# qzwlecr/p1

Hardware: AMD Instinct MI355X
Metric: SHA-256 nonce-hashes/sec (GH/s) (higher is better)
Workload: dtype u32

## Files before the change

include/p1hip.h:

```cpp
#ifndef P1HIP_H
#define P1HIP_H

#include <stddef.h>
#include <stdint.h>

#ifdef __cplusplus
extern "C" {
#endif

#define P1HIP_OK 0
#define P1HIP_ERR_NO_DEVICE (-1)
#define P1HIP_ERR_HIP (-2)
#define P1HIP_ERR_RCCL (-3)
#define P1HIP_ERR_ARGS (-4)

#define P1HIP_MAX_MSG_LEN ((size_t)1 << 28)

int p1hip_init(int want_devices, int *got_devices);

int p1hip_init_devices(const int *ordinals, int n);

int p1hip_scan(const uint8_t *msg, size_t msg_len, uint64_t lower, uint64_t upper,
               uint64_t *out_hash, uint64_t *out_nonce);

// ... 23 lines not shown
  uint64_t tiles;
  uint64_t nonces;
  double wall_ms;
} p1hip_batch_stats_t;
int p1hip_get_batch_stats(p1hip_batch_stats_t *out);

int p1hip_scan_batch_wide(const p1hip_request_t *reqs, size_t n, p1hip_result_t *out);

int p1hip_wide_layout(const p1hip_request_t *reqs, size_t n, int ndev,
                      int32_t *route, int32_t *device, uint32_t *segs, uint32_t *tiles);

int p1hip_wide_ranges(const p1hip_request_t *reqs, size_t n, int ndev, size_t cap, size_t *count,
                      uint32_t *req, uint32_t *tile0, uint32_t *ntiles, int32_t *launch,
                      uint32_t *dev_tiles);

typedef struct {
  uint64_t calls;
  uint64_t requests;
  uint64_t empty;
  uint64_t small;
  uint64_t wide;
  uint64_t individual;
  uint64_t scan_launches;
  uint64_t scan_segments;
  uint64_t generic_launches;
  uint64_t generic_segments;
  uint64_t tiles;
  uint64_t nonces;
  double wall_ms;
} p1hip_wide_stats_t;
int p1hip_get_wide_stats(p1hip_wide_stats_t *out);

typedef struct {
  uint64_t scans;
  uint64_t fast_launches;
  uint64_t fast_nonces;
  uint64_t fast_alg_ops;
  uint64_t generic_launches;
  uint64_t generic_nonces;
  double scan_wall_ms;
  uint64_t scan_launches;
  uint64_t scan_nonces;
  uint64_t scan_alg_ops;
  double scan_kernel_ms;
  uint64_t small_scans;
  uint64_t table_replans;
} p1hip_stats_t;

typedef struct {
  int32_t ordinal;
  int32_t active;
  uint64_t shard_first;
  uint64_t shard_last;
  uint64_t scans;
  uint64_t scan_launches;
  uint64_t scan_nonces;
  uint64_t scan_alg_ops;
  double scan_kernel_ms;
  double phase1_ms;
  double gather_ms;
} p1hip_device_stats_t;

int p1hip_get_device_stats(int index, p1hip_device_stats_t *out);

int p1hip_set_profiling(int on);
int p1hip_get_stats(p1hip_stats_t *out);
// ... 34 lines not shown
```

p1_amd/__init__.py:

```python
from ._lib import (
    P1HipError,
    lib_path,
    load,
    init,
    init_devices,
    scan,
    scan_batch,
    batch_layout,
    get_batch_stats,
    scan_batch_wide,
    wide_layout,
    get_wide_stats,
    hash,
    reduce_pairs,
    plan_shards,
    set_profiling,
    get_stats,
    get_device_stats,
    reset_stats,
    device_count,
    device_info,
    comm_info,
    abi_version,
    ABI_VERSION,
    test_knobs,
    shutdown,
    version,
    codeobj_bytes,
    codeobj_sha256,
    batch_codeobj_sha256,
)
from .sharding import shard_range, combine_keys
```

p1_amd/_lib.py:

```python
import ctypes
import os

_HERE = os.path.dirname(os.path.abspath(__file__))
_LIB = None

U64 = ctypes.c_uint64


class P1HipError(RuntimeError):
    def __init__(self, rc, msg):
        super().__init__(f"p1hip rc={rc}: {msg}")
        self.rc = rc


class Stats(ctypes.Structure):
    _fields_ = [
        ("scans", U64),
        ("fast_launches", U64),
        ("fast_nonces", U64),
        ("fast_alg_ops", U64),
        ("generic_launches", U64),
        ("generic_nonces", U64),
        ("scan_wall_ms", ctypes.c_double),
        ("scan_launches", U64),
# ... 38 lines not shown
class BatchStats(ctypes.Structure):
    _fields_ = [
        ("calls", U64),
        ("requests", U64),
        ("coalesced", U64),
        ("individual", U64),
        ("empty", U64),
        ("launches", U64),
        ("tiles", U64),
        ("nonces", U64),
        ("wall_ms", ctypes.c_double),
    ]

    def as_dict(self):
        return {k: getattr(self, k) for k, _ in self._fields_}


class WideStats(ctypes.Structure):
    _fields_ = [
        ("calls", U64),
        ("requests", U64),
        ("empty", U64),
        ("small", U64),
        ("wide", U64),
        ("individual", U64),
        ("scan_launches", U64),
        ("scan_segments", U64),
        ("generic_launches", U64),
        ("generic_segments", U64),
        ("tiles", U64),
        ("nonces", U64),
        ("wall_ms", ctypes.c_double),
    ]

    def as_dict(self):
        return {k: getattr(self, k) for k, _ in self._fields_}


class DeviceInfo(ctypes.Structure):
    _fields_ = [
        ("ordinal", ctypes.c_int32),
        ("cu_count", ctypes.c_int32),
        ("clock_khz", ctypes.c_int32),
        ("reserved", ctypes.c_int32),
        ("hbm_bytes", U64),
        ("pci_bus_id", ctypes.c_char * 32),
        ("arch", ctypes.c_char * 32),
        ("uuid", ctypes.c_ubyte * 16),
    ]

    def as_dict(self):
        return {"ordinal": self.ordinal, "cu_count": self.cu_count, "clock_khz": self.clock_khz,
                "hbm_bytes": self.hbm_bytes, "pci_bus_id": self.pci_bus_id.decode(errors="replace"),
                "arch": self.arch.decode(errors="replace"), "uuid": bytes(self.uuid).hex()}


def lib_path():
    return os.environ.get("P1HIP_LIB") or os.path.join(_HERE, "libp1hip.so")


SIGNATURES = [
    ("p1hip_init", ctypes.c_int, [ctypes.c_int, ctypes.POINTER(ctypes.c_int)]),
    ("p1hip_init_devices", ctypes.c_int, [ctypes.POINTER(ctypes.c_int), ctypes.c_int]),
    ("p1hip_scan", ctypes.c_int,
     [ctypes.c_char_p, ctypes.c_size_t, U64, U64, ctypes.POINTER(U64), ctypes.POINTER(U64)]),
    ("p1hip_scan_batch", ctypes.c_int, [ctypes.POINTER(Request), ctypes.c_size_t, ctypes.POINTER(Result)]),
    ("p1hip_batch_layout", ctypes.c_int,
     [ctypes.POINTER(Request), ctypes.c_size_t, ctypes.c_int, ctypes.POINTER(ctypes.c_uint32),
      ctypes.POINTER(ctypes.c_int32), ctypes.POINTER(ctypes.c_int32)]),
    ("p1hip_get_batch_stats", ctypes.c_int, [ctypes.POINTER(BatchStats)]),
    ("p1hip_scan_batch_wide", ctypes.c_int, [ctypes.POINTER(Request), ctypes.c_size_t, ctypes.POINTER(Result)]),
    ("p1hip_wide_layout", ctypes.c_int,
     [ctypes.POINTER(Request), ctypes.c_size_t, ctypes.c_int, ctypes.POINTER(ctypes.c_int32),
      ctypes.POINTER(ctypes.c_int32), ctypes.POINTER(ctypes.c_uint32), ctypes.POINTER(ctypes.c_uint32)]),
    ("p1hip_wide_ranges", ctypes.c_int,
     [ctypes.POINTER(Request), ctypes.c_size_t, ctypes.c_int, ctypes.c_size_t, ctypes.POINTER(ctypes.c_size_t),
      ctypes.POINTER(ctypes.c_uint32), ctypes.POINTER(ctypes.c_uint32), ctypes.POINTER(ctypes.c_uint32),
      ctypes.POINTER(ctypes.c_int32), ctypes.POINTER(ctypes.c_uint32)]),
    ("p1hip_get_wide_stats", ctypes.c_int, [ctypes.POINTER(WideStats)]),
    ("p1hip_hash", ctypes.c_int, [ctypes.c_char_p, ctypes.c_size_t, U64, ctypes.POINTER(U64)]),
    ("p1hip_plan_shards", ctypes.c_int,
     [ctypes.c_char_p, ctypes.c_size_t, U64, U64, ctypes.c_int, ctypes.POINTER(U64), ctypes.POINTER(U64)]),
    ("p1hip_reduce_pairs", ctypes.c_int,
     [ctypes.POINTER(U64), ctypes.POINTER(U64), ctypes.c_size_t, ctypes.POINTER(U64), ctypes.POINTER(U64)]),
    ("p1hip_set_profiling", ctypes.c_int, [ctypes.c_int]),
    ("p1hip_get_stats", ctypes.c_int, [ctypes.POINTER(Stats)]),
    ("p1hip_reset_stats", None, []),
    ("p1hip_get_device_stats", ctypes.c_int, [ctypes.c_int, ctypes.POINTER(DeviceStats)]),
    ("p1hip_device_count", ctypes.c_int, []),
    ("p1hip_device_info", ctypes.c_int, [ctypes.c_int, ctypes.POINTER(DeviceInfo)]),
    ("p1hip_comm_info", ctypes.c_int, [ctypes.c_int, ctypes.POINTER(ctypes.c_int), ctypes.POINTER(ctypes.c_int)]),
    ("p1hip_abi_version", ctypes.c_int, []),
    ("p1hip_test_knobs", ctypes.c_char_p, []),
    ("p1hip_last_error", ctypes.c_char_p, []),
    ("p1hip_version", ctypes.c_char_p, []),
    ("p1hip_shutdown", None, []),
]


def load(path=None):
    global _LIB
    if _LIB is not None and path is None:
        return _LIB
    p = path or lib_path()
    if not os.path.exists(p):
        raise P1HipError(-100, f"{p} not built (run `make` or __graft_entry__.build())")
    lib = ctypes.CDLL(p)
    for name, res, args in SIGNATURES:
        fn = getattr(lib, name)
        fn.restype = res
        fn.argtypes = args
    if lib.p1hip_abi_version() != ABI_VERSION:
# ... 82 lines not shown
    _check(load().p1hip_wide_layout(arr, n, int(ndev), route, device, segs, tiles))
    lay = [{"route": WIDE_ROUTES[route[i]], "device": device[i], "segs": segs[i], "tiles": tiles[i], "ranges": []}
           for i in range(n)]
    cap = sum(x["segs"] + 1 for x in lay)
    count = ctypes.c_size_t(0)
    req, tile0, ntiles = ((ctypes.c_uint32 * max(cap, 1))() for _ in range(3))
    launch = (ctypes.c_int32 * max(cap, 1))()
    dev_tiles = (ctypes.c_uint32 * int(ndev))()
    _check(load().p1hip_wide_ranges(arr, n, int(ndev), cap, ctypes.byref(count), req, tile0, ntiles, launch,
                                    dev_tiles))
    assert count.value <= cap
    for j in range(count.value):
        lay[req[j]]["ranges"].append((tile0[j], ntiles[j], launch[j]))
    return lay, list(dev_tiles)


def get_wide_stats():
    s = WideStats()
    _check(load().p1hip_get_wide_stats(ctypes.byref(s)))
    return s.as_dict()


def batch_codeobj_sha256(lib=None):
    import hashlib

    lib = lib or load()
    start = ctypes.addressof(ctypes.c_char.in_dll(lib, "p1hip_batch_co"))
    end = ctypes.addressof(ctypes.c_char.in_dll(lib, "p1hip_batch_co_end"))
    if end <= start:
        raise P1HipError(-100, "embedded batch code object is empty")
    return hashlib.sha256(ctypes.string_at(start, end - start)).hexdigest()


def hash(msg, nonce):
    m = _bytes(msg)
    h = U64()
    _check(load().p1hip_hash(m, len(m), int(nonce), ctypes.byref(h)))
    return h.value


def plan_shards(msg, lower, upper, n):
    m = _bytes(msg)
    first, last = (U64 * n)(), (U64 * n)()
    _check(load().p1hip_plan_shards(m, len(m), int(lower), int(upper), int(n), first, last))
    return [(a, b) if a <= b else None for a, b in zip(first, last)]


def reduce_pairs(hashes, nonces):
    n = len(hashes)
    assert n == len(nonces)
    ha = (U64 * max(n, 1))(*hashes)
    na = (U64 * max(n, 1))(*nonces)
    h, o = U64(), U64()
    _check(load().p1hip_reduce_pairs(ha, na, n, ctypes.byref(h), ctypes.byref(o)))
    return h.value, o.value


def set_profiling(on):
    _check(load().p1hip_set_profiling(1 if on else 0))


def get_stats():
    s = Stats()
    _check(load().p1hip_get_stats(ctypes.byref(s)))
    return s.as_dict()

# ... 61 lines not shown
```

p1_amd/csrc/p1hip.hip:

```cpp
#include <hip/hip_runtime.h>
#include <rccl/rccl.h>

#include <stdlib.h>
#include <string.h>

#include <algorithm>
#include <atomic>
#include <chrono>
#include <exception>
#include <mutex>
#include <string>
#include <thread>
#include <utility>
#include <vector>

#include "../../include/p1hip.h"
#include "batch_plan.hpp"
#include "planner.hpp"
#include "scan_abi.hpp"
#include "scan_pack.hpp"
#include "wide_plan.hpp"

extern "C" const unsigned char p1hip_kernels_co[];
extern "C" const unsigned char p1hip_batch_co[];

using namespace p1;

namespace {

thread_local std::string g_err;

int fail(int rc, const std::string& what) {
  g_err = what;
  return rc;
}

template <typename Fn>
int guarded(Fn&& fn) {
  try {
    return fn();
  } catch (const std::exception& ex) {
    return fail(P1HIP_ERR_HIP, std::string("host: ") + ex.what());
  } catch (...) {
    return fail(P1HIP_ERR_HIP, "host: unknown exception");
  }
}

#define HIPCHK(expr)                                                                        \
  do {                                                                                      \
    hipError_t e_ = (expr);                                                                 \
    if (e_ != hipSuccess)                                                                   \
      return fail(P1HIP_ERR_HIP, std::string(#expr) + ": " + hipGetErrorString(e_));       \
  } while (0)

#define NCCLCHK(expr)                                                                       \
  do {                                                                                      \
    ncclResult_t r_ = (expr);                                                               \
    if (r_ != ncclSuccess)                                                                  \
      return fail(P1HIP_ERR_RCCL, std::string(#expr) + ": " + ncclGetErrorString(r_));      \
  } while (0)

constexpr size_t kMaxKwTabs = 8;
constexpr uint64_t kMaxKwTabBytes = 8ull << 30;
constexpr uint64_t kMaxScanSpan = 1ull << 40;

enum KnobKind { kValue, kZeroDef, kFlag };
enum KnobWhen { kPerScan, kPerBatch, kAtInit };
enum KnobId {
  kSmallMaxNoncesKnob, kMaxLaunchBlocksKnob, kMaxScanSpanKnob, kKwtabMaxBytesKnob, kNoRcclKnob, kForceRcclKnob,
  kMinFastThreadsKnob, kTestFailDeviceKnob, kNoTableKnob, kNoSplitKnob, kScanGridKnob, kBatchMaxNoncesKnob,
  kBatchMaxTilesKnob, kWideMaxNoncesKnob, kWideMaxSegsKnob, kWideMinFastThreadsKnob, kKnobCount
};
struct Knob {
  const char* name;
  uint64_t def, max;
  KnobKind kind;
  KnobWhen when;
  const char* what;
};
const Knob kKnobs[] = {
    {"P1HIP_SMALL_MAX_NONCES", kSmallMaxNonces, kSmallMaxNonces, kValue, kPerScan,
     "shares of at most this many nonces take the one-launch small path; 0 turns it off, so small parity ranges "
     "run the fast kernel variants"},
    {"P1HIP_MAX_LAUNCH_BLOCKS", kMaxLaunchBlocks, kMaxLaunchBlocks, kZeroDef, kPerScan,
     "workgroups per k_scan launch, so GPU tests run the multi-launch path on small ranges; a larger piece gets "
     "a launch of its own (at most kMaxFastThreads / kBlock = 2^18 workgroups, far below HIP's grid limit)"},
    {"P1HIP_MAX_SCAN_SPAN", kMaxScanSpan, ~0ull, kZeroDef, kPerScan, "nonces per piece of a device's share"},
    {"P1HIP_KWTAB_MAX_BYTES", kMaxKwTabBytes, ~0ull, kValue, kPerScan,
     "MODE 5 table cap; a larger table re-plans the share without MODE 5"},
    {"P1HIP_NO_RCCL", 0, 1, kFlag, kAtInit,
     "combine the per-device results through the host, so the multi-device path (threads, sharding, combine) "
     "runs with the same GPU listed twice on a 1-GPU box"},
    {"P1HIP_FORCE_RCCL", 0, 1, kFlag, kAtInit, "a communicator even for one device"},
    {"P1HIP_MIN_FAST_THREADS", kMinFastThreads, ~0ull, kValue, kAtInit,
     "planner occupancy floor; 1 keeps k = 3 on small ranges so every k = 3 variant runs on the GPU"},
    {"P1HIP_TEST_FAIL_DEVICE", ~0ull, ~0ull, kValue, kAtInit,
     "device index whose scan phase reports a failure (the multi-device error path); default -1: none"},
    {"P1HIP_NO_TABLE", 0, 1, kFlag, kAtInit,
     "no MODE 5: layouts whose tail block 1 holds only lo digits run the digit-update variants (A/B, and a "
     "second kernel path to cross-check MODE 5)"},
    {"P1HIP_NO_SPLIT", 0, 1, kFlag, kAtInit,
     "straddling lo digits use mode 2 instead of the split modes (A/B builds with -DP1_NV2_PLAIN)"},
    {"P1HIP_SCAN_GRID", 0, kMaxLaunchBlocks, kZeroDef, kPerScan,
     "k_scan's grid instead of the device's workgroup slots (the default, 0); at or above a launch's tile count "
     "every workgroup runs one tile and the queue hands out none (the round-5 dispatch, same code object)"},
    {"P1HIP_BATCH_MAX_NONCES", kBatchMaxNonces, kBatchMaxNonces, kValue, kPerBatch,
     "requests of at most this many nonces are coalesced by p1hip_scan_batch; 0 runs every request "
     "individually; independent of P1HIP_SMALL_MAX_NONCES"},
    {"P1HIP_BATCH_MAX_TILES", kBatchMaxTiles, kBatchMaxTiles, kZeroDef, kPerBatch,
     "tiles per launch pair, so GPU tests run several launch pairs on small batches (batch_layout raises it to "
     "the largest single request's tile count)"},
    {"P1HIP_WIDE_MAX_NONCES", kWideMaxNonces, kWideMaxNonces, kValue, kPerBatch,
     "requests above the coalescing limit and of at most this many nonces share k_scan launches in "
     "p1hip_scan_batch_wide; larger ones run individually (0: all of them)"},
    {"P1HIP_WIDE_MAX_SEGS", kMaxSegs, kMaxSegs, kZeroDef, kPerBatch,
     "segments per k_scan launch of p1hip_scan_batch_wide, so GPU tests run many launches back to back on small "
     "calls and requests whose pieces land in different launches"},
    {"P1HIP_WIDE_MIN_FAST_THREADS", 0, ~0ull, kZeroDef, kPerBatch,
     "occupancy floor the wide requests are planned with instead of wide_min_fast_threads' rule (the default, "
     "0); 1 keeps k = 3"},
};
static_assert(sizeof kKnobs / sizeof kKnobs[0] == kKnobCount, "one row per KnobId, in its order");

bool test_knobs_on() {
  const char* m = getenv("P1HIP_TEST_KNOBS");
  return m && m[0] == '1' && m[1] == 0;
}

const char* test_knob(const char* name) {
  if (!test_knobs_on()) return nullptr;
  const char* v = getenv(name);
  return v && *v ? v : nullptr;
}

uint64_t knob(KnobId id) {
  const Knob& K = kKnobs[id];
  const char* v = test_knob(K.name);
  if (!v) return K.def;
  if (K.kind == kFlag) return v[0] == '1';
  const uint64_t n = strtoull(v, nullptr, 10);
  if (n == 0 && K.kind == kZeroDef) return K.def;
  return n < K.max ? n : K.max;
}

template <typename T, bool kPinned>
struct Buf {
  T* p = nullptr;
  size_t cap = 0;

  Buf() = default;
  Buf(const Buf&) = delete;
  Buf(Buf&& o) noexcept : p(std::exchange(o.p, nullptr)), cap(std::exchange(o.cap, 0)) {}
  Buf& operator=(Buf&& o) noexcept {
    if (this != &o) {
      (void)release();
      p = std::exchange(o.p, nullptr);
      cap = std::exchange(o.cap, 0);
    }
    return *this;
  }
  ~Buf() { (void)release(); }

  hipError_t release() {
    hipError_t e = hipSuccess;
    if (p) e = kPinned ? hipHostFree(p) : hipFree(p);
    p = nullptr;
    cap = 0;
    return e;
  }
  hipError_t reserve(size_t need, size_t floor, size_t extra = 0) {
    if (need <= cap) return hipSuccess;
    hipError_t e = release();
    if (e != hipSuccess) return e;
    size_t n = floor;
    while (n < need) n <<= 1;
    const size_t bytes = (n + extra) * sizeof(T);
    e = kPinned ? hipHostMalloc(&p, bytes, hipHostMallocDefault) : hipMalloc(&p, bytes);
    if (e != hipSuccess) p = nullptr;
    else cap = n;
    return e;
  }
};
template <typename T> using DevBuf = Buf<T, false>;
template <typename T> using PinnedBuf = Buf<T, true>;

struct Dev {
  int ordinal = -1;
  hipStream_t stream = nullptr;
  DevBuf<Key> d_part;
  DevBuf<Key> d_res;
  DevBuf<Key> d_gather;
  PinnedBuf<Key> h_res;
  DevBuf<Segment> d_seg;
  PinnedBuf<Segment> h_seg;
  ncclComm_t comm = nullptr;
  hipModule_t mod = nullptr;
  hipFunction_t f_scan = nullptr, f_reduce = nullptr, f_pairs = nullptr, f_small = nullptr, f_kwtable = nullptr;
  DevBuf<Key> d_small_part;
  DevBuf<uint32_t> d_ticket;
  DevBuf<uint32_t> d_scan_ticket;
  uint32_t scan_grid = 0;
  bool small_used = false;
  hipModule_t bmod = nullptr;
  hipFunction_t f_bscan = nullptr, f_breduce = nullptr, f_wreduce = nullptr;
  DevBuf<BatchSeg> d_bseg;
  PinnedBuf<BatchSeg> h_bseg;
  DevBuf<uint32_t> d_btile0;
  PinnedBuf<uint32_t> h_btile0;
  DevBuf<Key> d_bout;
  PinnedBuf<Key> h_bout;
  DevBuf<Key> d_bpart;
  DevBuf<WideRange> d_wrange;
  PinnedBuf<WideRange> h_wrange;
  std::vector<hipEvent_t> evs;
  struct KwTab {
    uint32_t w[16];
    int k;
    uint32_t* dptr;
    uint64_t used_in;
  };
  std::vector<KwTab> kwtabs;
  uint64_t range_id = 0;
  ScanCounters ctr;
  uint64_t replans = 0;
  p1hip_device_stats_t acc{};
};

struct Runtime {
  std::mutex mu;
  std::vector<Dev> devs;
  bool profiling = false;
  bool use_rccl = true;
  bool rccl_one = false;
  uint64_t min_fast_threads = kMinFastThreads;
  bool split = true;
  bool tabulate = true;
  int fail_device = -1;
  p1hip_stats_t stats{};
  p1hip_batch_stats_t bstats{};
  p1hip_wide_stats_t wstats{};
};

Runtime& rt() {
  static Runtime* r = new Runtime();
  return *r;
}

int device_count(int* count) {
  *count = 0;
  if (hipGetDeviceCount(count) != hipSuccess || *count <= 0)
    return fail(P1HIP_ERR_NO_DEVICE, "no HIP device visible");
  return P1HIP_OK;
}

template <typename... Args>
hipError_t launch(hipFunction_t f, uint32_t blocks, uint32_t threads, hipStream_t st, Args... args) {
  void* params[] = {(void*)&args...};
  return hipModuleLaunchKernel(f, blocks, 1, 1, threads, 1, 1, 0, st, params, nullptr);
}

int ev_record(Dev& d, size_t& nev) {
  if (d.evs.size() <= nev) {
    hipEvent_t e;
    HIPCHK(hipEventCreate(&e));
    d.evs.push_back(e);
  }
  HIPCHK(hipEventRecord(d.evs[nev], d.stream));
  ++nev;
  return P1HIP_OK;
}

int ev_sum(Dev& d, size_t nev) {
  if (!nev) return P1HIP_OK;
// ... 11 lines not shown
  return k;
}

void add_counters(p1hip_stats_t& s, const ScanCounters& c) {
  s.fast_launches += c.fast_launches;
  s.fast_nonces += c.fast_nonces;
  s.fast_alg_ops += c.fast_ops;
  s.generic_launches += c.gen_launches;
  s.generic_nonces += c.gen_nonces;
  s.scan_launches += c.scan_launches;
  s.scan_nonces += c.scan_nonces;
  s.scan_alg_ops += c.scan_ops;
  s.scan_kernel_ms += c.scan_ms;
}

void add_counters(p1hip_device_stats_t& a, const ScanCounters& c) {
  a.scans++;
  a.scan_launches += c.scan_launches;
  a.scan_nonces += c.scan_nonces;
  a.scan_alg_ops += c.scan_ops;
  a.scan_kernel_ms += c.scan_ms;
}

int dev_release(Dev& d) {
  if (d.ordinal < 0) return 0;
  (void)hipSetDevice(d.ordinal);
  if (d.stream) (void)hipStreamSynchronize(d.stream);
  for (hipEvent_t e : d.evs) (void)hipEventDestroy(e);
  for (Dev::KwTab& t : d.kwtabs) (void)hipFree(t.dptr);
  if (d.comm) ncclCommDestroy(d.comm);
  if (d.stream) (void)hipStreamDestroy(d.stream);
  if (d.mod) (void)hipModuleUnload(d.mod);
  if (d.bmod) (void)hipModuleUnload(d.bmod);
  d = Dev();
  return 0;
}

void shutdown_locked(Runtime& R) {
  for (Dev& d : R.devs) dev_release(d);
  R.devs.clear();
}

int init_devs(Runtime& R, const std::vector<int>& ords) {
  int count = 0;
  if (int rc = device_count(&count)) return rc;
  const int nd = (int)ords.size();
  std::vector<int> cus(ords.size());
  for (int i = 0; i < nd; ++i) {
    const int o = ords[i];
    if (o < 0 || o >= count) return fail(P1HIP_ERR_NO_DEVICE, "device ordinal out of range: " + std::to_string(o));
    hipDeviceProp_t prop;
    HIPCHK(hipGetDeviceProperties(&prop, o));
    if (std::string(prop.gcnArchName).rfind("gfx950", 0) != 0)
      return fail(P1HIP_ERR_NO_DEVICE, std::string("device is not gfx950: ") + prop.gcnArchName);
    cus[i] = prop.multiProcessorCount;
  }
  R.devs.resize(ords.size());
  for (int i = 0; i < nd; ++i) {
    Dev& d = R.devs[i];
    d.ordinal = ords[i];
    HIPCHK(hipSetDevice(d.ordinal));
    HIPCHK(hipStreamCreateWithFlags(&d.stream, hipStreamNonBlocking));
    HIPCHK(hipModuleLoadData(&d.mod, p1hip_kernels_co));
    HIPCHK(hipModuleGetFunction(&d.f_scan, d.mod, "k_scan"));
    HIPCHK(hipModuleGetFunction(&d.f_reduce, d.mod, "k_reduce"));
    HIPCHK(hipModuleGetFunction(&d.f_pairs, d.mod, "k_pairs"));
    HIPCHK(hipModuleGetFunction(&d.f_small, d.mod, "k_scan_small"));
    HIPCHK(hipModuleGetFunction(&d.f_kwtable, d.mod, "k_kwtable"));
    HIPCHK(hipModuleLoadData(&d.bmod, p1hip_batch_co));
    HIPCHK(hipModuleGetFunction(&d.f_bscan, d.bmod, "k_batch_scan"));
    HIPCHK(hipModuleGetFunction(&d.f_breduce, d.bmod, "k_batch_reduce"));
    HIPCHK(hipModuleGetFunction(&d.f_wreduce, d.bmod, "k_wide_reduce"));
    HIPCHK(d.d_small_part.reserve(kSmallMaxBlocks, kSmallMaxBlocks));
    HIPCHK(d.d_ticket.reserve(1, 1));
    HIPCHK(d.d_scan_ticket.reserve(2, 2));
    HIPCHK(hipMemsetAsync(d.d_ticket.p, 0, sizeof(uint32_t), d.stream));
    HIPCHK(hipMemsetAsync(d.d_scan_ticket.p, 0, 2 * sizeof(uint32_t), d.stream));
    int per_cu = 0;
    HIPCHK(hipModuleOccupancyMaxActiveBlocksPerMultiprocessor(&per_cu, d.f_scan, kBlock, 0));
    if (per_cu < 1 || cus[i] < 1)
      return fail(P1HIP_ERR_HIP, "k_scan occupancy: " + std::to_string(per_cu) + " blocks per CU");
    d.scan_grid = (uint32_t)per_cu * (uint32_t)cus[i];
    HIPCHK(hipStreamSynchronize(d.stream));
    HIPCHK(d.d_res.reserve(1, 1));
    HIPCHK(d.d_gather.reserve((size_t)nd, (size_t)nd));
    HIPCHK(d.h_res.reserve((size_t)nd, (size_t)nd));
  }
  R.use_rccl = !knob(kNoRcclKnob);
  R.rccl_one = knob(kForceRcclKnob) && R.use_rccl;
  R.min_fast_threads = knob(kMinFastThreadsKnob);
  R.split = !knob(kNoSplitKnob);
  R.tabulate = !knob(kNoTableKnob);
  R.fail_device = (int)(int64_t)knob(kTestFailDeviceKnob);
  if ((nd > 1 || R.rccl_one) && R.use_rccl) {
    std::vector<ncclComm_t> comms(nd);
    NCCLCHK(ncclCommInitAll(comms.data(), nd, ords.data()));
    for (int i = 0; i < nd; ++i) R.devs[i].comm = comms[i];
  }
  return P1HIP_OK;
}

int init_locked(Runtime& R, const std::vector<int>& ords) {
  if (!R.devs.empty()) {
    bool same = R.devs.size() == ords.size();
    for (size_t i = 0; same && i < ords.size(); ++i) same = R.devs[i].ordinal == ords[i];
    if (same) return P1HIP_OK;
    shutdown_locked(R);
  }
  const int rc = init_devs(R, ords);
  if (rc != P1HIP_OK) {
    const std::string keep = g_err;
    shutdown_locked(R);
    g_err = keep;
  }
  return rc;
// ... 54 lines not shown
    if (v == d.kwtabs.size()) return kNoTable;
    HIPCHK(hipFree(d.kwtabs[v].dptr));
    d.kwtabs.erase(d.kwtabs.begin() + (long)v);
  }
  Dev::KwTab t;
  memcpy(t.w, L.tabw, sizeof t.w);
  t.k = L.tabk;
  t.dptr = nullptr;
  t.used_in = d.range_id;
  const uint32_t rows = (uint32_t)pow10u(L.tabk);
  const hipError_t me = hipMalloc(&t.dptr, (size_t)rows * 64u * sizeof(uint32_t));
  if (me == hipErrorOutOfMemory) {
    (void)hipGetLastError();
    return kNoTable;
  }
  HIPCHK(me);
  KwTableArgs a;
  memset(&a, 0, sizeof a);
  memcpy(a.tabw, L.tabw, sizeof a.tabw);
  a.k = (uint32_t)L.tabk;
  a.qv = (uint32_t)(L.Y.q - 64);
  a.rows = rows;
  a.out = t.dptr;
  const hipError_t e = launch(d.f_kwtable, (rows + kBlock - 1) / kBlock, kBlock, d.stream, a);
  if (e != hipSuccess) {
    (void)hipFree(t.dptr);
    return fail(P1HIP_ERR_HIP, std::string("k_kwtable launch: ") + hipGetErrorString(e));
  }
  d.kwtabs.push_back(t);
  *dptr = (uint64_t)(uintptr_t)t.dptr;
  return P1HIP_OK;
}

uint32_t scan_grid_for(const Dev& d, uint32_t tiles) {
  const uint64_t g = knob(kScanGridKnob);
  return std::min(tiles, g > 0 ? (uint32_t)g : d.scan_grid);
}

int run_range(Dev& d, const uint8_t* msg, size_t len, uint64_t lo, uint64_t hi, bool profiling,
              uint64_t min_fast_threads, bool split, bool tabulate) {
  HIPCHK(hipSetDevice(d.ordinal));
  d.range_id++;
  d.ctr = {};
  Plan plan;
  std::vector<uint64_t> tabptr;
  for (;;) {
    std::string err = make_plan(msg, len, lo, hi, plan, true, min_fast_threads, split, tabulate);
    if (!err.empty()) return fail(P1HIP_ERR_ARGS, "planner: " + err);
    tabptr.assign(plan.launches.size(), 0);
    bool replan = false;
    for (size_t i = 0; i < plan.launches.size() && !replan; ++i) {
      const Launch& L = plan.launches[i];
      if (!L.fast || (L.mode != 5 && L.mode != 7)) continue;
      const int rt = kwtable_for(d, L, &tabptr[i]);
      if (rt == kNoTable) replan = true;
      else if (rt != P1HIP_OK) return rt;
    }
    if (!replan) break;
    tabulate = false;
    d.replans++;
    plan = Plan();
  }
  const ScanPack P = pack_scan(plan, knob(kMaxLaunchBlocksKnob));
  HIPCHK(d.d_part.reserve(P.total_blocks, 1));
  HIPCHK(d.d_seg.reserve(P.batches.size() * kMaxSegs, 4 * kMaxSegs));
  HIPCHK(d.h_seg.reserve(P.batches.size() * kMaxSegs, 4 * kMaxSegs));
  int rc;
  size_t nev = 0;
  uint32_t part_off = 0;
  for (size_t bi = 0; bi < P.batches.size(); ++bi) {
    const ScanBatch& B = P.batches[bi];
    Segment* hs = d.h_seg.p + bi * kMaxSegs;
    Segment* ds = d.d_seg.p + bi * kMaxSegs;
    const std::string err = fill_segments(plan, P, B, tabptr.data(), hs, d.ctr);
    if (!err.empty()) return fail(P1HIP_ERR_ARGS, err);
    HIPCHK(hipMemcpyAsync(ds, hs, B.count * sizeof(Segment), hipMemcpyHostToDevice, d.stream));
    if (profiling && (rc = ev_record(d, nev))) return rc;
#ifdef P1_STATIC_GRID
    HIPCHK(launch(d.f_scan, B.blocks, kBlock, d.stream, (const Segment*)ds, (uint32_t)B.count,
                  (Key*)(d.d_part.p + part_off)));
#else
    HIPCHK(launch(d.f_scan, scan_grid_for(d, B.blocks), kBlock, d.stream, (const Segment*)ds,
                  (uint32_t)B.count, (Key*)(d.d_part.p + part_off), (uint32_t)B.blocks, d.d_scan_ticket.p));
#endif
    if (profiling && (rc = ev_record(d, nev))) return rc;
    part_off += B.blocks;
  }
  HIPCHK(launch(d.f_reduce, 1, kReduceThreads, d.stream, (const Key*)d.d_part.p, P.total_blocks, d.d_res.p));
  return ev_sum(d, nev);
}

int run_share(Dev& d, const uint8_t* msg, size_t len, uint64_t lo, uint64_t hi, const Runtime& R) {
  const uint64_t span = knob(kMaxScanSpanKnob);
  if (hi - lo < span)
    return run_range(d, msg, len, lo, hi, R.profiling, R.min_fast_threads, R.split, R.tabulate);
  Key best = {~0ull, ~0ull};
  ScanCounters sum;
  for (uint64_t a = lo;;) {
    const uint64_t b = hi - a < span ? hi : a + (span - 1);
    int r = run_range(d, msg, len, a, b, R.profiling, R.min_fast_threads, R.split, R.tabulate);
    if (r != P1HIP_OK) return r;
    Key k;
    HIPCHK(hipMemcpyAsync(&k, d.d_res.p, sizeof(Key), hipMemcpyDeviceToHost, d.stream));
    HIPCHK(hipStreamSynchronize(d.stream));
    if (key_lt(k, best)) best = k;
    sum += d.ctr;
    if (b == hi) break;
    a = b + 1;
  }
  d.ctr = sum;
  HIPCHK(hipMemcpyAsync(d.d_res.p, &best, sizeof(Key), hipMemcpyHostToDevice, d.stream));
  HIPCHK(hipStreamSynchronize(d.stream));
  return P1HIP_OK;
}

// ... 35 lines not shown
    auto run_phase = [&](double p1hip_device_stats_t::*ms, auto&& body) {
      run_threads([&](size_t i) {
        Dev& d = R.devs[i];
        const auto p0 = std::chrono::steady_clock::now();
        int r;
        try {
          r = body(i, d);
        } catch (const std::exception& ex) {
          try {
            r = fail(P1HIP_ERR_HIP, std::string("host: ") + ex.what());
          } catch (...) {
            r = P1HIP_ERR_HIP;
          }
        } catch (...) {
          r = P1HIP_ERR_HIP;
        }
        d.acc.*ms += std::chrono::duration<double, std::milli>(std::chrono::steady_clock::now() - p0).count();
        rcs[i] = r;
        if (r) {
          try {
            errs[i] = g_err;
          } catch (...) {
          }
        }
      });
      for (size_t i = 0; i < nd; ++i)
        if (rcs[i]) return fail(rcs[i], "device " + std::to_string(R.devs[i].ordinal) + ": " + errs[i]);
      return (int)P1HIP_OK;
    };
    const bool coll = (nd > 1 || R.rccl_one) && R.use_rccl;
    const uint64_t small_max = knob(kSmallMaxNoncesKnob);
    rc = run_phase(&p1hip_device_stats_t::phase1_ms, [&](size_t i, Dev& d) -> int {
      d.ctr = {};
      d.replans = 0;
      d.small_used = false;
      d.acc.shard_first = slo[i];
      d.acc.shard_last = shi[i];
      d.acc.active = active[i];
      int r = P1HIP_OK;
      if ((int)i == R.fail_device) {
        r = fail(P1HIP_ERR_HIP, "injected failure (P1HIP_TEST_FAIL_DEVICE)");
      } else if (active[i] && shi[i] - slo[i] < small_max) {
        d.small_used = true;
        r = run_small(d, msg, msg_len, slo[i], shi[i], !coll && nd == 1, R.profiling);
      } else if (active[i]) {
        r = run_share(d, msg, msg_len, slo[i], shi[i], R);
      } else {
        if (hipSetDevice(d.ordinal) != hipSuccess) r = fail(P1HIP_ERR_HIP, "hipSetDevice");
        if (!r && hipMemsetAsync(d.d_res.p, 0xFF, sizeof(Key), d.stream) != hipSuccess)
          r = fail(P1HIP_ERR_HIP, "hipMemsetAsync(identity)");
      }
      if (!r && !coll && nd > 1) {
        if (hipMemcpyAsync(R.devs[0].h_res.p + i, d.d_res.p, sizeof(Key), hipMemcpyDeviceToHost, d.stream) !=
            hipSuccess)
          r = fail(P1HIP_ERR_HIP, "hipMemcpyAsync(result)");
      } else if (!r && !coll && !(active[i] && d.small_used)) {
        if (hipMemcpyAsync(d.h_res.p, d.d_res.p, sizeof(Key), hipMemcpyDeviceToHost, d.stream) != hipSuccess)
          r = fail(P1HIP_ERR_HIP, "hipMemcpyAsync(result)");
      }
      if (!r && hipStreamSynchronize(d.stream) != hipSuccess) r = fail(P1HIP_ERR_HIP, "hipStreamSynchronize");
      return r;
    });
    if (rc != P1HIP_OK) return rc;
    if (coll) {
      rc = run_phase(&p1hip_device_stats_t::gather_ms, [&](size_t i, Dev& d) -> int {
        if (hipSetDevice(d.ordinal) != hipSuccess) return fail(P1HIP_ERR_HIP, "hipSetDevice");
        ncclResult_t nr = ncclAllGather(d.d_res.p, d.d_gather.p, 2, ncclUint64, d.comm, d.stream);
        if (nr != ncclSuccess) return fail(P1HIP_ERR_RCCL, std::string("ncclAllGather: ") + ncclGetErrorString(nr));
        if (i == 0 &&
            hipMemcpyAsync(d.h_res.p, d.d_gather.p, sizeof(Key) * nd, hipMemcpyDeviceToHost, d.stream) != hipSuccess)
          return fail(P1HIP_ERR_HIP, "hipMemcpyAsync(gathered)");
        if (hipStreamSynchronize(d.stream) != hipSuccess) return fail(P1HIP_ERR_HIP, "hipStreamSynchronize");
        return P1HIP_OK;
      });
      if (rc != P1HIP_OK) return rc;
    }
    Key b = {~0ull, ~0ull};
    for (size_t i = 0; i < nd; ++i) b = key_lt(R.devs[0].h_res.p[i], b) ? R.devs[0].h_res.p[i] : b;
    res = finish_key(b);
    for (Dev& d : R.devs) {
      add_counters(R.stats, d.ctr);
      add_counters(d.acc, d.ctr);
      if (d.small_used && d.ctr.scan_launches) R.stats.small_scans++;
      R.stats.table_replans += d.replans;
    }
  }
  R.stats.scans++;
  R.stats.scan_wall_ms +=
      std::chrono::duration<double, std::milli>(std::chrono::steady_clock::now() - t0).count();
  *out_hash = res.h;
  *out_nonce = res.n;
  return P1HIP_OK;
}

int scan_locked(const uint8_t* msg, size_t msg_len, uint64_t lower, uint64_t upper, uint64_t* out_hash,
                uint64_t* out_nonce) {
  Runtime& R = rt();
  std::lock_guard<std::mutex> g(R.mu);
  return scan_held(R, msg, msg_len, lower, upper, out_hash, out_nonce);
}

int batch_check(const p1hip_request_t* reqs, size_t n) {
  for (size_t i = 0; i < n; ++i) {
    if (!reqs[i].msg && reqs[i].msg_len > 0)
      return fail(P1HIP_ERR_ARGS, "request " + std::to_string(i) + ": msg == NULL with msg_len > 0");
    if (reqs[i].msg_len > P1HIP_MAX_MSG_LEN)
      return fail(P1HIP_ERR_ARGS, "request " + std::to_string(i) + ": msg_len exceeds P1HIP_MAX_MSG_LEN");
  }
  return P1HIP_OK;
}

std::vector<BatchReq> batch_reqs(const p1hip_request_t* reqs, size_t n) {
  std::vector<BatchReq> q(n);
  for (size_t i = 0; i < n; ++i) q[i] = {reqs[i].msg, reqs[i].msg_len, reqs[i].lower, reqs[i].upper};
  return q;
}

// ... 423 lines not shown

int p1hip_hash(const uint8_t* msg, size_t msg_len, uint64_t nonce, uint64_t* out_hash) {
  uint64_t n = 0;
  return p1hip_scan(msg, msg_len, nonce, nonce, out_hash, &n);
}

int p1hip_reduce_pairs(const uint64_t* hashes, const uint64_t* nonces, size_t n, uint64_t* out_hash,
                       uint64_t* out_nonce) {
  if (!out_hash || !out_nonce || (n && (!hashes || !nonces))) return fail(P1HIP_ERR_ARGS, "null pointer");
  return guarded([&]() { return reduce_pairs_locked(hashes, nonces, n, out_hash, out_nonce); });
}

int p1hip_set_profiling(int on) {
  Runtime& R = rt();
  std::lock_guard<std::mutex> g(R.mu);
  R.profiling = on != 0;
  return P1HIP_OK;
}

int p1hip_get_stats(p1hip_stats_t* out) {
  if (!out) return fail(P1HIP_ERR_ARGS, "null stats pointer");
  Runtime& R = rt();
  std::lock_guard<std::mutex> g(R.mu);
  *out = R.stats;
  return P1HIP_OK;
}

void p1hip_reset_stats(void) {
  Runtime& R = rt();
  std::lock_guard<std::mutex> g(R.mu);
  R.stats = p1hip_stats_t{};
  R.bstats = p1hip_batch_stats_t{};
  R.wstats = p1hip_wide_stats_t{};
  for (Dev& d : R.devs) {
    d.acc = p1hip_device_stats_t{};
    d.acc.shard_first = 1;
  }
}

int p1hip_get_device_stats(int index, p1hip_device_stats_t* out) {
  if (!out) return fail(P1HIP_ERR_ARGS, "null stats pointer");
  Runtime& R = rt();
  std::lock_guard<std::mutex> g(R.mu);
  if (index < 0 || (size_t)index >= R.devs.size()) return fail(P1HIP_ERR_ARGS, "device index out of range");
  *out = R.devs[(size_t)index].acc;
  out->ordinal = R.devs[(size_t)index].ordinal;
  return P1HIP_OK;
}

int p1hip_comm_info(int index, int* nranks, int* rank) {
  if (!nranks || !rank) return fail(P1HIP_ERR_ARGS, "null comm-info pointer");
  *nranks = 0;
  *rank = -1;
  Runtime& R = rt();
  std::lock_guard<std::mutex> g(R.mu);
  if (index < 0 || (size_t)index >= R.devs.size()) return fail(P1HIP_ERR_ARGS, "device index out of range");
  const Dev& d = R.devs[(size_t)index];
  if (!d.comm) return P1HIP_OK;
  int count = 0, user = -1;
  NCCLCHK(ncclCommCount(d.comm, &count));
  NCCLCHK(ncclCommUserRank(d.comm, &user));
  *nranks = count;
  *rank = user;
  return P1HIP_OK;
}

int p1hip_abi_version(void) { return P1HIP_ABI_VERSION; }

const char* p1hip_last_error(void) { return g_err.c_str(); }

// ... 68 lines not shown
```

p1_amd/csrc/scan_pack.hpp:

```cpp
#pragma once
#include <string.h>

#include <algorithm>
#include <string>
#include <vector>

#include "planner.hpp"
#include "scan_abi.hpp"

namespace p1 {

constexpr uint32_t kMaxSegs = 64;
constexpr uint32_t kMaxLaunchBlocks = 1u << 22;

inline bool has_variant(int fv, int mode, bool trail) {
#define P1_CASE(FV, MODE, TR) \
  if (fv == FV && mode == MODE && trail == TR) return true;
#include "fast_variants.inc"
#undef P1_CASE
  return false;
}

struct ScanCounters {
  uint64_t fast_launches = 0, fast_nonces = 0, fast_ops = 0, gen_launches = 0, gen_nonces = 0;
// ... 15 lines not shown

struct ScanPack {
  std::vector<size_t> order;
  std::vector<ScanBatch> batches;
  uint32_t total_blocks = 0;
};

inline ScanPack pack_scan(const Plan& plan, uint64_t max_blocks, uint32_t max_segs = kMaxSegs) {
  ScanPack P;
  P.order.resize(plan.launches.size());
  for (size_t i = 0; i < P.order.size(); ++i) P.order[i] = i;
  auto weight = [&](size_t i) -> uint64_t {
    const Launch& L = plan.launches[i];
    return L.fast ? (uint64_t)(L.fa.kpow / L.fa.nsub) * (uint64_t)L.btail : (uint64_t)L.btail - 1;
  };
  std::stable_sort(P.order.begin(), P.order.end(), [&](size_t a, size_t b) { return weight(a) > weight(b); });
  uint64_t all_blocks = 0;
  for (const Launch& L : plan.launches) all_blocks += L.blocks;
  const uint64_t nlaunch = (all_blocks + max_blocks - 1) / max_blocks;
  const uint64_t target = nlaunch > 1 ? (all_blocks + nlaunch - 1) / nlaunch : max_blocks;
  for (size_t r = 0; r < P.order.size(); ++r) {
    const Launch& L = plan.launches[P.order[r]];
    const uint64_t cur = P.batches.empty() ? 0 : P.batches.back().blocks;
    if (P.batches.empty() || P.batches.back().count == max_segs || cur + (uint64_t)L.blocks > max_blocks ||
        (cur > 0 && cur + L.blocks / 2 > target && P.batches.size() < nlaunch))
      P.batches.push_back({r, 0, 0});
    P.batches.back().count++;
    P.batches.back().blocks += L.blocks;
    P.total_blocks += L.blocks;
  }
  return P;
}

inline std::string fill_segments(const Plan& plan, const ScanPack& P, const ScanBatch& B, const uint64_t* tabptr,
                                 Segment* segs, ScanCounters& c) {
  uint32_t block0 = 0;
  for (size_t j = 0; j < B.count; ++j) {
    const size_t i = P.order[B.first + j];
    const Launch& L = plan.launches[i];
    Segment& S = segs[j];
    memset(&S, 0, sizeof S);
    S.block0 = block0;
    block0 += L.blocks;
    if (L.fast) {
      if (!has_variant(L.fv, L.mode, L.trail)) return "no fast kernel variant";
      S.kind = variant_id(L.fv, L.mode, L.trail);
      S.fa = L.fa;
      if (L.mode == 5 || L.mode == 7) S.fa.kwtab = tabptr[i];
      c.fast_launches++;
      c.fast_nonces += L.nonces;
      c.fast_ops += L.nonces * kAlgOpsPerCompression * (uint64_t)L.btail;
    } else {
      S.kind = kGenericKind;
      S.ga = L.ga;
      c.gen_launches++;
      c.gen_nonces += L.nonces;
    }
    c.scan_nonces += L.nonces;
    c.scan_ops += L.nonces * kAlgOpsPerCompression * (uint64_t)L.btail;
  }
  c.scan_launches++;
  return "";
}

inline std::string fill_small(const Plan& plan, SmallArgs& a, ScanCounters& c) {
  if (plan.launches.size() > kSmallMaxSegs || plan.total_blocks > kSmallMaxBlocks)
// ... 21 lines not shown
```

Measured before the change: 54.58.

## Add alternate tab scan code object chosen per batch for table-mode launches

Embeds a second compiled code object of the scan kernels, built without MachineLICM and post-processed to hoist constants. Each scan batch is routed to it when most of its nonces come from fast mode-5 table launches with k at least 5, and it gets its own occupancy-derived grid size. This is meant to cut register pressure or spills that hoisting adds in the table-heavy kernels. The cost is an extra module load per device, more build complexity, and a per-batch selection heuristic that could choose the slower object.

New measurement: 54.58, median of 4. About the same (-0.0%).

```diff
diff --git a/include/p1hip.h b/include/p1hip.h
--- a/include/p1hip.h
+++ b/include/p1hip.h
@@ -79,6 +79,14 @@
 int p1hip_get_wide_stats(p1hip_wide_stats_t *out);
 
 typedef struct {
+  uint64_t main_launches;
+  uint64_t main_nonces;
+  uint64_t tab_launches;
+  uint64_t tab_nonces;
+} p1hip_scan_object_stats_t;
+int p1hip_get_scan_object_stats(p1hip_scan_object_stats_t *out);
+
+typedef struct {
   uint64_t scans;
   uint64_t fast_launches;
   uint64_t fast_nonces;
diff --git a/p1_amd/__init__.py b/p1_amd/__init__.py
--- a/p1_amd/__init__.py
+++ b/p1_amd/__init__.py
@@ -29,5 +29,8 @@
     codeobj_bytes,
     codeobj_sha256,
     batch_codeobj_sha256,
+    tab_codeobj_bytes,
+    tab_codeobj_sha256,
+    get_scan_object_stats,
 )
 from .sharding import shard_range, combine_keys
diff --git a/p1_amd/_lib.py b/p1_amd/_lib.py
--- a/p1_amd/_lib.py
+++ b/p1_amd/_lib.py
@@ -94,6 +94,13 @@
         ("nonces", U64),
         ("wall_ms", ctypes.c_double),
     ]
+
+    def as_dict(self):
+        return {k: getattr(self, k) for k, _ in self._fields_}
+
+
+class ScanObjectStats(ctypes.Structure):
+    _fields_ = [("main_launches", U64), ("main_nonces", U64), ("tab_launches", U64), ("tab_nonces", U64)]
 
     def as_dict(self):
         return {k: getattr(self, k) for k, _ in self._fields_}
@@ -140,6 +147,7 @@
       ctypes.POINTER(ctypes.c_uint32), ctypes.POINTER(ctypes.c_uint32), ctypes.POINTER(ctypes.c_uint32),
       ctypes.POINTER(ctypes.c_int32), ctypes.POINTER(ctypes.c_uint32)]),
     ("p1hip_get_wide_stats", ctypes.c_int, [ctypes.POINTER(WideStats)]),
+    ("p1hip_get_scan_object_stats", ctypes.c_int, [ctypes.POINTER(ScanObjectStats)]),
     ("p1hip_hash", ctypes.c_int, [ctypes.c_char_p, ctypes.c_size_t, U64, ctypes.POINTER(U64)]),
     ("p1hip_plan_shards", ctypes.c_int,
      [ctypes.c_char_p, ctypes.c_size_t, U64, U64, ctypes.c_int, ctypes.POINTER(U64), ctypes.POINTER(U64)]),
@@ -288,6 +296,27 @@
     return hashlib.sha256(ctypes.string_at(start, end - start)).hexdigest()
 
 
+def tab_codeobj_bytes(lib=None):
+    lib = lib or load()
+    start = ctypes.addressof(ctypes.c_char.in_dll(lib, "p1hip_tab_co"))
+    end = ctypes.addressof(ctypes.c_char.in_dll(lib, "p1hip_tab_co_end"))
+    if end <= start:
+        raise P1HipError(-100, "embedded tab code object is empty")
+    return ctypes.string_at(start, end - start)
+
+
+def tab_codeobj_sha256(lib=None):
+    import hashlib
+
+    return hashlib.sha256(tab_codeobj_bytes(lib)).hexdigest()
+
+
+def get_scan_object_stats():
+    s = ScanObjectStats()
+    _check(load().p1hip_get_scan_object_stats(ctypes.byref(s)))
+    return s.as_dict()
+
+
 def hash(msg, nonce):
     m = _bytes(msg)
     h = U64()
diff --git a/p1_amd/csrc/p1hip.hip b/p1_amd/csrc/p1hip.hip
--- a/p1_amd/csrc/p1hip.hip
+++ b/p1_amd/csrc/p1hip.hip
@@ -23,6 +23,7 @@
 
 extern "C" const unsigned char p1hip_kernels_co[];
 extern "C" const unsigned char p1hip_batch_co[];
+extern "C" const unsigned char p1hip_tab_co[];
 
 using namespace p1;
 
@@ -69,7 +70,7 @@
 enum KnobId {
   kSmallMaxNoncesKnob, kMaxLaunchBlocksKnob, kMaxScanSpanKnob, kKwtabMaxBytesKnob, kNoRcclKnob, kForceRcclKnob,
   kMinFastThreadsKnob, kTestFailDeviceKnob, kNoTableKnob, kNoSplitKnob, kScanGridKnob, kBatchMaxNoncesKnob,
-  kBatchMaxTilesKnob, kWideMaxNoncesKnob, kWideMaxSegsKnob, kWideMinFastThreadsKnob, kKnobCount
+  kBatchMaxTilesKnob, kWideMaxNoncesKnob, kWideMaxSegsKnob, kWideMinFastThreadsKnob, kScanObjectKnob, kKnobCount
 };
 struct Knob {
   const char* name;
@@ -119,6 +120,9 @@
     {"P1HIP_WIDE_MIN_FAST_THREADS", 0, ~0ull, kZeroDef, kPerBatch,
      "occupancy floor the wide requests are planned with instead of wide_min_fast_threads' rule (the default, "
      "0); 1 keeps k = 3"},
+    {"P1HIP_SCAN_OBJECT", 0, 0, kValue, kPerScan,
+     "main or tab: the scan object of every k_scan launch of p1hip_scan instead of scan_object_of's choice (read "
+     "as text by forced_scan_object, not through knob())"},
 };
 static_assert(sizeof kKnobs / sizeof kKnobs[0] == kKnobCount, "one row per KnobId, in its order");
 
@@ -141,6 +145,14 @@
   const uint64_t n = strtoull(v, nullptr, 10);
   if (n == 0 && K.kind == kZeroDef) return K.def;
   return n < K.max ? n : K.max;
+}
+
+int forced_scan_object() {
+  const char* v = test_knob(kKnobs[kScanObjectKnob].name);
+  if (!v) return -1;
+  if (strcmp(v, "main") == 0) return kScanObjMain;
+  if (strcmp(v, "tab") == 0) return kScanObjTab;
+  return -1;
 }
 
 template <typename T, bool kPinned>
@@ -200,6 +212,11 @@
   DevBuf<uint32_t> d_ticket;
   DevBuf<uint32_t> d_scan_ticket;
   uint32_t scan_grid = 0;
+  hipModule_t tmod = nullptr;
+  hipFunction_t f_scan_tab = nullptr;
+  uint32_t scan_grid_tab = 0;
+  uint64_t obj_launches[kScanObjCount] = {0, 0};
+  uint64_t obj_nonces[kScanObjCount] = {0, 0};
   bool small_used = false;
   hipModule_t bmod = nullptr;
   hipFunction_t f_bscan = nullptr, f_breduce = nullptr, f_wreduce = nullptr;
@@ -239,6 +256,7 @@
   p1hip_stats_t stats{};
   p1hip_batch_stats_t bstats{};
   p1hip_wide_stats_t wstats{};
+  p1hip_scan_object_stats_t ostats{};
 };
 
 Runtime& rt() {
@@ -316,6 +334,7 @@
   if (d.stream) (void)hipStreamDestroy(d.stream);
   if (d.mod) (void)hipModuleUnload(d.mod);
   if (d.bmod) (void)hipModuleUnload(d.bmod);
+  if (d.tmod) (void)hipModuleUnload(d.tmod);
   d = Dev();
   return 0;
 }
@@ -365,6 +384,13 @@
     if (per_cu < 1 || cus[i] < 1)
       return fail(P1HIP_ERR_HIP, "k_scan occupancy: " + std::to_string(per_cu) + " blocks per CU");
     d.scan_grid = (uint32_t)per_cu * (uint32_t)cus[i];
+    HIPCHK(hipModuleLoadData(&d.tmod, p1hip_tab_co));
+    HIPCHK(hipModuleGetFunction(&d.f_scan_tab, d.tmod, "k_scan_tab"));
+    per_cu = 0;
+    HIPCHK(hipModuleOccupancyMaxActiveBlocksPerMultiprocessor(&per_cu, d.f_scan_tab, kBlock, 0));
+    if (per_cu < 1)
+      return fail(P1HIP_ERR_HIP, "k_scan_tab occupancy: " + std::to_string(per_cu) + " blocks per CU");
+    d.scan_grid_tab = (uint32_t)per_cu * (uint32_t)cus[i];
     HIPCHK(hipStreamSynchronize(d.stream));
     HIPCHK(d.d_res.reserve(1, 1));
     HIPCHK(d.d_gather.reserve((size_t)nd, (size_t)nd));
@@ -485,9 +511,9 @@
   return P1HIP_OK;
 }
 
-uint32_t scan_grid_for(const Dev& d, uint32_t tiles) {
+uint32_t scan_grid_for(const Dev& d, uint32_t tiles, int obj = kScanObjMain) {
   const uint64_t g = knob(kScanGridKnob);
-  return std::min(tiles, g > 0 ? (uint32_t)g : d.scan_grid);
+  return std::min(tiles, g > 0 ? (uint32_t)g : obj == kScanObjTab ? d.scan_grid_tab : d.scan_grid);
 }
 
 int run_range(Dev& d, const uint8_t* msg, size_t len, uint64_t lo, uint64_t hi, bool profiling,
@@ -515,6 +541,7 @@
     plan = Plan();
   }
   const ScanPack P = pack_scan(plan, knob(kMaxLaunchBlocksKnob));
+  const int forced = forced_scan_object();
   HIPCHK(d.d_part.reserve(P.total_blocks, 1));
   HIPCHK(d.d_seg.reserve(P.batches.size() * kMaxSegs, 4 * kMaxSegs));
   HIPCHK(d.h_seg.reserve(P.batches.size() * kMaxSegs, 4 * kMaxSegs));
@@ -525,15 +552,20 @@
     const ScanBatch& B = P.batches[bi];
     Segment* hs = d.h_seg.p + bi * kMaxSegs;
     Segment* ds = d.d_seg.p + bi * kMaxSegs;
+    const uint64_t nonces0 = d.ctr.scan_nonces;
     const std::string err = fill_segments(plan, P, B, tabptr.data(), hs, d.ctr);
     if (!err.empty()) return fail(P1HIP_ERR_ARGS, err);
+    const int obj = forced >= 0 ? forced : (int)scan_object_of(plan, P, B);
+    const hipFunction_t f_scan = obj == kScanObjTab ? d.f_scan_tab : d.f_scan;
+    d.obj_launches[obj]++;
+    d.obj_nonces[obj] += d.ctr.scan_nonces - nonces0;
     HIPCHK(hipMemcpyAsync(ds, hs, B.count * sizeof(Segment), hipMemcpyHostToDevice, d.stream));
     if (profiling && (rc = ev_record(d, nev))) return rc;
 #ifdef P1_STATIC_GRID
-    HIPCHK(launch(d.f_scan, B.blocks, kBlock, d.stream, (const Segment*)ds, (uint32_t)B.count,
+    HIPCHK(launch(f_scan, B.blocks, kBlock, d.stream, (const Segment*)ds, (uint32_t)B.count,
                   (Key*)(d.d_part.p + part_off)));
 #else
-    HIPCHK(launch(d.f_scan, scan_grid_for(d, B.blocks), kBlock, d.stream, (const Segment*)ds,
+    HIPCHK(launch(f_scan, scan_grid_for(d, B.blocks, obj), kBlock, d.stream, (const Segment*)ds,
                   (uint32_t)B.count, (Key*)(d.d_part.p + part_off), (uint32_t)B.blocks, d.d_scan_ticket.p));
 #endif
     if (profiling && (rc = ev_record(d, nev))) return rc;
@@ -635,6 +667,7 @@
     const uint64_t small_max = knob(kSmallMaxNoncesKnob);
     rc = run_phase(&p1hip_device_stats_t::phase1_ms, [&](size_t i, Dev& d) -> int {
       d.ctr = {};
+      for (int o = 0; o < kScanObjCount; ++o) d.obj_launches[o] = d.obj_nonces[o] = 0;
       d.replans = 0;
       d.small_used = false;
       d.acc.shard_first = slo[i];
@@ -686,6 +719,10 @@
       add_counters(d.acc, d.ctr);
       if (d.small_used && d.ctr.scan_launches) R.stats.small_scans++;
       R.stats.table_replans += d.replans;
+      R.ostats.main_launches += d.obj_launches[kScanObjMain];
+      R.ostats.main_nonces += d.obj_nonces[kScanObjMain];
+      R.ostats.tab_launches += d.obj_launches[kScanObjTab];
+      R.ostats.tab_nonces += d.obj_nonces[kScanObjTab];
     }
   }
   R.stats.scans++;
@@ -1175,10 +1212,19 @@
   R.stats = p1hip_stats_t{};
   R.bstats = p1hip_batch_stats_t{};
   R.wstats = p1hip_wide_stats_t{};
+  R.ostats = p1hip_scan_object_stats_t{};
   for (Dev& d : R.devs) {
     d.acc = p1hip_device_stats_t{};
     d.acc.shard_first = 1;
   }
+}
+
+int p1hip_get_scan_object_stats(p1hip_scan_object_stats_t* out) {
+  if (!out) return fail(P1HIP_ERR_ARGS, "null stats pointer");
+  Runtime& R = rt();
+  std::lock_guard<std::mutex> g(R.mu);
+  *out = R.ostats;
+  return P1HIP_OK;
 }
 
 int p1hip_get_device_stats(int index, p1hip_device_stats_t* out) {
diff --git a/p1_amd/csrc/p1hip_tab_blob.S b/p1_amd/csrc/p1hip_tab_blob.S
--- /dev/null
+++ b/p1_amd/csrc/p1hip_tab_blob.S
@@ -0,0 +1,16 @@
+/* Embeds the "tab" scan object (Makefile: build/p1hip_tab.hsaco, the scan
+   kernels of p1hip_kernels.hip compiled without MachineLICM and post-passed
+   with --hoist-consts
+   the scan object of p1hip_kernels_blob.S and the batch object of
+   p1hip_batch_blob.S
+   on every device it initialises and launches it where scan_pack.hpp
+   scan_object_of picks it. */
+    .section .rodata
+    .balign 4096
+    .globl p1hip_tab_co
+    .type p1hip_tab_co, @object
+p1hip_tab_co:
+    .incbin P1HIP_TAB_CO
+    .globl p1hip_tab_co_end
+p1hip_tab_co_end:
+    .section .note.GNU-stack,"",@progbits
diff --git a/p1_amd/csrc/scan_pack.hpp b/p1_amd/csrc/scan_pack.hpp
--- a/p1_amd/csrc/scan_pack.hpp
+++ b/p1_amd/csrc/scan_pack.hpp
@@ -71,6 +71,20 @@
   return P;
 }
 
+enum ScanObject { kScanObjMain = 0, kScanObjTab = 1, kScanObjCount = 2 };
+inline const char* scan_object_name(int o) { return o == kScanObjTab ? "tab" : "main"; }
+constexpr int kTabObjMinK = 5;
+
+inline ScanObject scan_object_of(const Plan& plan, const ScanPack& P, const ScanBatch& B) {
+  uint64_t all = 0, tab = 0;
+  for (size_t j = 0; j < B.count; ++j) {
+    const Launch& L = plan.launches[P.order[B.first + j]];
+    all += L.nonces;
+    if (L.fast && L.mode == 5 && L.tabk >= kTabObjMinK) tab += L.nonces;
+  }
+  return tab > all - tab ? kScanObjTab : kScanObjMain;
+}
+
 inline std::string fill_segments(const Plan& plan, const ScanPack& P, const ScanBatch& B, const uint64_t* tabptr,
                                  Segment* segs, ScanCounters& c) {
   uint32_t block0 = 0;
```
